# fnordware/j2k

Hardware: AMD Instinct MI355X
Metric: Mpixels/s encode, 8Kx8K 16-bit RGB, 5 DWT levels; DWT HBM GB/s vs roofline (higher is better)
Workload: dtype f32

## Files before the change

j2k_amd/csrc/t1.hip:

```cpp
#include "kernels.h"
#include "t1_common.h"
#include "cblk_style.h"
#include "t1_mq_window.h"

#include <algorithm>
#include <cstdlib>
#include <type_traits>

namespace j2k_hip {
namespace {


constexpr int kFrac = 6;
constexpr int kFlush = 1024;
constexpr int kStageBytes = kFlush + 64 * 10;


__device__ __forceinline__ void set_priority(int p)
{
    if (p >= 3) __builtin_amdgcn_s_setprio(3);
    else if (p == 2) __builtin_amdgcn_s_setprio(2);
    else if (p == 1) __builtin_amdgcn_s_setprio(1);
}

// ... 474 lines not shown
                }
                const unsigned bitsh = hf(bits), Nh = hf(A) & ~hf(O), Vh = hf(V64);
                const bool any_rl = __any(rl != 0);
                unsigned fills = 0;
                if (any_rl) {
                    unsigned nof = Nh | (Nh >> 1);
                    nof = (nof | (nof >> 2) | ~rl) & 0x11111111u;
                    int wv = w;
                    asm volatile("" : "+s"(wv));
                    if (lane >= wv) nof = 0;
#define J2K_OR_STEP(ctrl, rmask) nof |= (unsigned)__builtin_amdgcn_update_dpp(0, (int)nof, ctrl, rmask, 0xf, false);
                    J2K_OR_STEP(0x111, 0xf) J2K_OR_STEP(0x112, 0xf) J2K_OR_STEP(0x114, 0xf) J2K_OR_STEP(0x118, 0xf)
                    J2K_OR_STEP(0x142, 0xa) J2K_OR_STEP(0x143, 0xc)
#undef J2K_OR_STEP
                    fills = active & ~(unsigned)__builtin_amdgcn_readlane((int)nof, 63);
                    DADD(48, __builtin_popcount(fills));
                    if (fills == active) DCNT(49);
                }
                bool sparse = false;
                u64 q0 = 0, q1 = 0;
                unsigned sparse_total = 0;
                if (a.sparse >= 0 && !any_rl) {
                    const unsigned dense_cost = kDenseStripe * (unsigned)__builtin_popcount(active);
                    if (a.sparse > 0 || !__any(kSparseHead + kSparseRound * (unsigned)__builtin_popcount(Vh) >= dense_cost)) {
                        const unsigned c = nibble_counts(Vh) + nibble_counts(Nh);
                        const unsigned c0 = c & 0x000f000fu, c1 = (c >> 4) & 0x000f000fu, c2 = (c >> 8) & 0x000f000fu, c3 = (c >> 12) & 0x000f000fu;
                        unsigned t0, t1, t2, t3;
                        const unsigned e0 = prefix_count_dpp(c0, t0), e1 = prefix_count_dpp(c1, t1), e2 = prefix_count_dpp(c2, t2), e3 = prefix_count_dpp(c3, t3);
                        const unsigned a1 = t0 + t1, a2 = a1 + t2, a3 = a2 + t3;
                        const unsigned total = (a3 & 0xffffu) + (a3 >> 16);
                        if (total <= kBurst) {
                            sparse = true;
                            sparse_total = total;
                            DCNT(pt == 0 ? 7 : 8);
                            DADD(pt == 0 ? 14 : 15, total);
                            const unsigned org = (fill - flushed) * 0x10001u + (a3 << 16);
                            q0 = (u64)(e0 + org) | ((u64)(e1 + org + t0) << 32);
                            q1 = (u64)(e2 + org + a1) | ((u64)(e3 + org + a2) << 32);
                        } else DCNT(17);
                    }
                }
                unsigned zb0 = 0, zb1 = 0, zb2 = 0, zb3 = 0, sb0 = 0, sb1 = 0, sb2 = 0, sd = 0;
                if (fills != active) {
                    const unsigned Wm1 = hf(LA << 1), W0 = hf(LA), Wp1 = hf(((LA >> 1) & ~M3) | (LO >> 1));
                    const unsigned Em1 = hf((RO << 1) | ((RA << 1) & M0)), E0 = hf(RO), Ep1 = hf(RO >> 1);
                    const unsigned Up = hf(A << 1), Dn = hf(O >> 1);
                    {
                        unsigned h1 = W0 ^ E0, h2 = W0 & E0, v1 = Up ^ Dn, v2 = Up & Dn;
                        if (orient == 1) { const unsigned t1 = h1, t2 = h2; h1 = v1; h2 = v2; v1 = t1; v2 = t2; }
                        const unsigned p = Wm1 ^ Wp1, q = Wm1 & Wp1, r_ = Em1 ^ Ep1, t = Em1 & Ep1;
                        const unsigned dodd = p ^ r_, dge1 = p | q | r_ | t, dge2 = (p & r_) | q | t;
                        const unsigned deq1 = dodd & ~dge2;
                        const unsigned hz = ~(h1 | h2), vnz = v1 | v2;
                        if (orient == 3) {
                            const unsigned dge3 = (q & (r_ | t)) | (t & p);
                            const unsigned deq2 = dge2 & ~dge3, deq0 = ~dge1;
                            const unsigned hv0 = hz & ~vnz, hv1 = (h1 & ~vnz) | (hz & v1), hvge2 = ~(hv0 | hv1);
                            zb3 = dge3;
                            zb2 = deq2 | (deq1 & ~hv0);
                            zb1 = deq2 | (deq1 & hv0) | (deq0 & hvge2);
                            zb0 = (deq2 & ~hv0) | (deq1 & (hv0 | hvge2)) | (deq0 & hv1);
                        } else {
                            zb3 = h2;
                            zb2 = h1 | (hz & v2);
                            zb1 = (h1 & (vnz | dge1)) | (hz & (v1 | (~vnz & dge2)));
                            zb0 = (h1 & (vnz | ~dge1)) | (hz & (v1 | (~vnz & deq1)));
                        }
                    }
                    if (any_n) {
                        const unsigned cL = hf(from_left64(chi)), cR = hf(from_right64(chi)), cU = hf(chi << 1), cD = hf(chi >> 1);
                        const unsigned Wp = W0 & ~cL, Wn = W0 & cL, Ep = E0 & ~cR, En = E0 & cR;
                        const unsigned Upp = Up & ~cU, Upn = Up & cU, Dnp = Dn & ~cD, Dnn = Dn & cD;
                        const unsigned hp = (Wp & ~En) | (Ep & ~Wn), hn = (Wn & ~Ep) | (En & ~Wp);
                        const unsigned vp = (Upp & ~Dnn) | (Dnp & ~Upn), vn = (Upn & ~Dnp) | (Dnn & ~Upp);
                        const unsigned hnz = hp | hn, vnz = vp | vn;
                        const unsigned same = (hp & vp) | (hn & vn), opp = (hp & vn) | (hn & vp);
                        sb2 = same;
                        sb1 = hnz & ~same;
                        sb0 = (hnz & ~same & ~opp) | (~hnz & vnz);
                        sd = hf(chi) ^ (hn | (~hnz & vn));
                        if constexpr (BYPASS) {
                            if (pt == 0 && pass >= 10) sd = hf(chi);
                        }
                    }
                }
                if (sparse) {
                    unsigned rest = Vh, pos = 0;
                    int cur = -1;
                    while (__any(rest != 0)) {
                        DCNT(9);
                        if (rest) {
                            const int r = __builtin_ctz(rest);
                            rest &= rest - 1;
                            const int st = r >> 2;
                            if (st != cur) pos = (unsigned)((r & 8 ? q1 : q0) >> (((r & 4) << 3) | (r & 16))) & 0xffffu;
                            cur = st;
                            const auto bit = [&](unsigned plane) { return __builtin_amdgcn_ubfe(plane, (unsigned)r, 1u); };
                            stage[pos] = (unsigned char)((((((((bit(zb3) << 1) | bit(zb2)) << 1) | bit(zb1)) << 1) | bit(zb0)) << 1) | bit(bitsh));
                            ++pos;
                            if (bit(Nh)) {
                                stage[pos] = (unsigned char)(0x12u + ((((((bit(sb2) << 1) | bit(sb1)) << 1) | bit(sb0)) << 1) | bit(sd)));
                                ++pos;
                            }
                        }
                    }
                    commit(sparse_total);
                    continue;
                }
                DCNT(pt == 0 ? 12 : 13);
                unsigned zi0e = 0, zi0o = 0, zi1e = 0, zi1o = 0;
                if (kPairTabs && fills != active) {
                    pair_index(bitsh, zb0, zi0e, zi0o);
                    pair_index(zb1, zb2, zi1e, zi1o);
                }
                while (active) {
                    const int sl = __builtin_ctz(active) & ~3;
                    active &= active - 1;
                    if ((fills >> sl) & 1u) {
                        int wv = w;
                        asm volatile("" : "+s"(wv));
                        if (lane < wv) stage[(fill - flushed) + lane] = (unsigned char)(CTX_RL << 1);
                        DADD(15, w);
                        commit((unsigned)w);
                        continue;
                    }
                    DCNT(pt == 0 ? 0 : 2);
                    const unsigned N = (Nh >> sl) & 0xfu;
                    unsigned Vz = (Vh >> sl) & 0xfu;
                    unsigned pc = 0, rlsym = 0;
                    if (pt != 0) {
                        if ((rl >> sl) & 1u) {
                            const int runlen = N ? __ffs((int)N) - 1 : 4;
                            rlsym = (CTX_RL << 1) | (runlen != 4 ? 1u : 0u);
                            pc = 1;
                            Vz = 0;
                            if (runlen != 4) {
                                rlsym |= (((CTX_UNI << 1) | (unsigned)(runlen >> 1)) << 8) | (((CTX_UNI << 1) | (unsigned)(runlen & 1)) << 16);
                                pc = 3;
                                Vz = 0xfu & ~((2u << runlen) - 1u);
                            }
                        }
                    }
                    const u64 sel = DIST ? kPackSel.v[Vz | (N << 4)] : sel_tab[Vz | (N << 4)];
                    const unsigned cnt = pc + (unsigned)__builtin_popcount(Vz) + (unsigned)__builtin_popcount(N);
                    unsigned total;
                    const unsigned base = reserve(cnt, std::integral_constant<int, 10>(), total);
                    unsigned zsym = 0, ssym = 0;
                    const auto nib = [&](unsigned plane) { return __builtin_amdgcn_ubfe(plane, (unsigned)sl, 4u); };
                    if constexpr (kPairTabs) {
                        const unsigned pick = 0x0c0c0c00u | ((unsigned)sl >> 3) | ((unsigned)sl & 4u);
                        if (__any(Vz != 0))
                            zsym = pair_entry(__builtin_amdgcn_perm(zi0o, zi0e, pick)) | (pair_entry(__builtin_amdgcn_perm(zi1o, zi1e, pick)) << 2) |
                                   (spread4(nib(zb3)) << 4);
                        if (__any(N != 0))
                            ssym = 0x12121212u + pair_entry(nib(sd) | (nib(sb0) << 4)) + (pair_entry(nib(sb1) | (nib(sb2) << 4)) << 2);
                    } else {
                        if (__any(Vz != 0))
                            zsym = (spread4(nib(zb0)) << 1) | (spread4(nib(zb1)) << 2) | (spread4(nib(zb2)) << 3) | (spread4(nib(zb3)) << 4) | spread4(nib(bitsh));
                        if (__any(N != 0))
                            ssym = 0x12121212u + (spread4(nib(sb0)) << 1) + (spread4(nib(sb1)) << 2) + (spread4(nib(sb2)) << 3) + spread4(nib(sd));
                    }
                    {
                        const unsigned c0 = __builtin_amdgcn_perm(ssym, zsym, (unsigned)sel), c1 = __builtin_amdgcn_perm(ssym, zsym, (unsigned)(sel >> 32));
                        const u64 d = (((u64)c1 << 32) | c0) << (8 * pc);
                        emit(base, cnt, (unsigned)d | rlsym, (unsigned)(d >> 32), __builtin_amdgcn_ubfe(c1, 8, 8 * pc));
                        DADD(pt == 0 ? 14 : 15, total);
                        commit(total);
                    }
                }
            }
            sigma = A;
            }
            }
            if (pt == 2) pi = 0;
            if constexpr (DIST) {
#pragma unroll
                for (int o = 32; o > 0; o >>= 1) nm += __shfl_xor(nm, o);
            }
            if (lane == 0) { pass_nsym[pass] = fill; pass_nmsedec[pass] = nm; }
            ++pass;
        }
    }
    __builtin_amdgcn_wave_barrier();
    const unsigned rest = fill - flushed;
    if (lane * 16u < rest) {
        if (flushed + lane * 16u + 16u <= symcap) {
            const uint4 v = *reinterpret_cast<const uint4 *>(&stage[lane * 16]);
            *reinterpret_cast<uint4 *>(symout + flushed + lane * 16) = v;
        } else overflow = true;
    }
#ifdef J2K_T1_COUNTERS
    if (lane == 0 && a.dbg) for (int i = 0; i < kT1Counters; ++i) if (dc[i]) atomicAdd(a.dbg + i, dc[i]);
#endif
    const bool ovf = __any(overflow);
    if (ovf && lane == 0) a.err[0] = 2u;
    if (lane == 0) { a.numbps[b] = (unsigned)numbps; a.npasses[b] = ovf ? 0u : (unsigned)pass; a.nsym[b] = ovf ? 0u : fill; }
    report();
}

constexpr unsigned mq2_slot(unsigned idx, unsigned mps, unsigned lps) { return idx | (mps << 6) | (lps << 7); }
constexpr unsigned kMq2LpsBit = 9;
constexpr bool mq2_slots_ok()
{
    bool seen[256] = {};
    for (unsigned idx = 0; idx < 47; ++idx)
        for (unsigned mps = 0; mps < 2; ++mps)
            for (unsigned lps = 0; lps < 2; ++lps) {
                const unsigned w = mq2_slot(idx, mps, lps), addr = w * 4u;
                if (w >= 256u || seen[w] || (addr & 3u) || (addr & ~0x3fcu)) return false;
                if (addr != ((mq2_slot(idx, mps, 0) * 4u) ^ (lps << kMq2LpsBit))) return false;
                seen[w] = true;
            }
    return true;
}
static_assert(mq2_slots_ok(), "trans: (index, sense, lps) -> word index must be injective over 47 x 2 x 2, below 256, and a word address within 0x3fc");
__device__ __forceinline__ unsigned ctx_word2(unsigned qe, unsigned idx, unsigned mps) { return (qe << 16) | (mq2_slot(idx, mps, 0) << 2) | (mps << kMq2LpsBit); }

#ifndef J2K_MQ2_RING
#define J2K_MQ2_RING 128
#endif
constexpr unsigned kRing = J2K_MQ2_RING;
template <bool RATES>
__global__ __launch_bounds__(128) void t1_mq2_kernel(T1Args a)
{
    __shared__ unsigned ctxs[19 * 64];
    __shared__ unsigned trans[256];
    __shared__ uint4 queue[2][4][64];
    __shared__ __attribute__((aligned(16))) unsigned ostage[(kRing / 4 + 1) * 64];
    __shared__ unsigned finalA[64];
    const int lane = threadIdx.x & 63;
    const bool producer = threadIdx.x < 64;
    __shared__ int gate_ok;
    T1Args::GateGroup gg{};
    bool gated_out = false;
    if (a.gate_groups) {
        gg = a.gate_groups[a.first + (int)blockIdx.x];
        if (threadIdx.x == 0) {
            unsigned polls = 0;
            int ok = 1;
            while (__hip_atomic_load(a.gate_ready + a.first + (int)blockIdx.x, __ATOMIC_ACQUIRE, __HIP_MEMORY_SCOPE_AGENT) < gg.count) {
                __builtin_amdgcn_s_sleep(127);
                if (++polls > a.gate_budget || (a.gate_abort && __hip_atomic_load(a.gate_abort, __ATOMIC_RELAXED, __HIP_MEMORY_SCOPE_AGENT))) { ok = 0; break; }
            }
            gate_ok = ok;
        }
        __syncthreads();
        __builtin_amdgcn_fence(__ATOMIC_ACQUIRE, "agent");
        gated_out = gate_ok == 0;
        if (gated_out && threadIdx.x == 0) a.err[0] = 4u;
        set_priority(a.mq_prio ? (int)gg.prio : 0);
    } else set_priority(a.mq_prio);
    const int b = a.gate_groups ? (int)gg.first + lane : a.first + (int)blockIdx.x * 64 + lane;
    if (producer) {
        if (lane < 47) {
            trans[mq2_slot(lane, 0, 0)] = ctx_word2(kQe[kNmps[lane]], kNmps[lane], 0);
            trans[mq2_slot(lane, 1, 0)] = ctx_word2(kQe[kNmps[lane]], kNmps[lane], 1);
            trans[mq2_slot(lane, 0, 1)] = ctx_word2(kQe[kNlps[lane]], kNlps[lane], kSwitch[lane]);
            trans[mq2_slot(lane, 1, 1)] = ctx_word2(kQe[kNlps[lane]], kNlps[lane], 1u ^ kSwitch[lane]);
        }
#pragma unroll
        for (int c = 0; c < 19; ++c) {
            const unsigned idx = c == CTX_UNI ? 46u : (c == CTX_RL ? 3u : (c == 0 ? 4u : 0u));
            ctxs[c * 64 + lane] = ctx_word2(kQe[idx], idx, 0);
        }
    }
    const bool live = a.gate_groups ? (lane < (int)gg.count && !gated_out) : b < a.nblks;
    CblkDev cb = {};
    unsigned nsym = 0, npasses = 0;
    if (live) { cb = a.blks[b]; nsym = a.nsym[b]; npasses = a.npasses[b]; }
    unsigned maxsym = nsym;
#pragma unroll
    for (int o = 32; o > 0; o >>= 1) maxsym = max(maxsym, (unsigned)__shfl_xor((int)maxsym, o));
    const unsigned nchunks = (unsigned)__builtin_amdgcn_readfirstlane((int)((maxsym + 15) / 16));
    __syncthreads();

    if (producer) {
        const unsigned char *sym = a.sym + cb.sym_off;
        unsigned A = 0x80000000u;
        uint4 next = make_uint4(0, 0, 0, 0);
        if (nsym) next = *reinterpret_cast<const uint4 *>(sym);
        unsigned yield_budget = 2048;
#ifdef J2K_MQ_TIMES
        long long tw_ = 0, tb_ = 0;
#endif
        for (unsigned c = 0; c <= nchunks; ++c) {
#ifdef J2K_MQ_TIMES
            const long long t0_ = __builtin_readcyclecounter();
#endif
            if (a.yield_word && (c & 3u) == 0) {
                while (yield_budget && __builtin_amdgcn_readfirstlane((int)__hip_atomic_load(a.yield_word, __ATOMIC_RELAXED, __HIP_MEMORY_SCOPE_AGENT))) {
                    __builtin_amdgcn_s_sleep(64);
                    --yield_budget;
                }
            }
            if (c < nchunks) {
                const unsigned base = c * 16;
                const uint4 chunk = next;
                if (base + 16 < nsym) next = *reinterpret_cast<const uint4 *>(sym + base + 16);
                const unsigned words[4] = {chunk.x, chunk.y, chunk.z, chunk.w};
                const int rem = (int)min(nsym - min(base, nsym), 16u);
                unsigned char *const ctx_b = reinterpret_cast<unsigned char *>(ctxs);
                const unsigned char *const trans_b = reinterpret_cast<const unsigned char *>(trans);
                const unsigned lane4 = (unsigned)lane * 4u;
                auto decide = [&](unsigned c4, unsigned b4, auto jj_) -> unsigned {
                    constexpr unsigned jj = decltype(jj_)::value;
                    unsigned *const cp = reinterpret_cast<unsigned *>(ctx_b + __builtin_amdgcn_perm(c4, lane4, 0x0c0c0400u + (jj << 8)));
                    const unsigned st = *cp;
                    const unsigned ta = (st ^ __builtin_amdgcn_perm(b4, 0u, 0x0c0c040cu + (jj << 8))) & 0x3fcu;
                    const unsigned tr = *reinterpret_cast<const unsigned *>(trans_b + ta);
                    const bool mps = ta < (1u << kMq2LpsBit);
                    const unsigned qe = st & 0xffff0000u;
                    const unsigned A1 = A - qe;
                    const bool use_a1 = (A1 >= qe) == mps;
                    A = use_a1 ? A1 : qe;
                    const bool renorm = (int)A >= 0;
                    *cp = renorm ? tr : st;
                    const unsigned n = (unsigned)__builtin_clz(A);
                    A <<= n;
                    return __builtin_amdgcn_alignbit(n, use_a1 ? qe : 0u, 16);
                };
                if (__all(rem == 16)) {
#pragma unroll
                    for (int g = 0; g < 4; ++g) {
                        const unsigned c4 = (words[g] >> 1) & 0x1f1f1f1fu, b4 = words[g] << 1;
                        unsigned e[4];
                        e[0] = decide(c4, b4, std::integral_constant<unsigned, 0>());
                        e[1] = decide(c4, b4, std::integral_constant<unsigned, 1>());
                        e[2] = decide(c4, b4, std::integral_constant<unsigned, 2>());
                        e[3] = decide(c4, b4, std::integral_constant<unsigned, 3>());
                        queue[c & 1][g][lane] = make_uint4(e[0], e[1], e[2], e[3]);
                    }
                } else
#pragma unroll
                for (int g = 0; g < 4; ++g) {
                    const unsigned c4 = (words[g] >> 1) & 0x1f1f1f1fu, b4 = words[g] << 1;
                    unsigned e[4] = {0, 0, 0, 0};
                    if (4 * g + 0 < rem) e[0] = decide(c4, b4, std::integral_constant<unsigned, 0>());
                    if (4 * g + 1 < rem) e[1] = decide(c4, b4, std::integral_constant<unsigned, 1>());
                    if (4 * g + 2 < rem) e[2] = decide(c4, b4, std::integral_constant<unsigned, 2>());
                    if (4 * g + 3 < rem) e[3] = decide(c4, b4, std::integral_constant<unsigned, 3>());
                    queue[c & 1][g][lane] = make_uint4(e[0], e[1], e[2], e[3]);
                }
            } else {
                finalA[lane] = A >> 16;
            }
#ifdef J2K_MQ_TIMES
            const long long t1_ = __builtin_readcyclecounter();
            __syncthreads();
            tw_ += t1_ - t0_; tb_ += __builtin_readcyclecounter() - t1_;
#else
            __syncthreads();
#endif
        }
#ifdef J2K_MQ_TIMES
        if (lane == 0 && a.dbg) { atomicAdd(a.dbg + 0, (unsigned long long)tw_); atomicAdd(a.dbg + 1, (unsigned long long)tb_); atomicAdd(a.dbg + 4, (unsigned long long)nchunks); atomicAdd(a.dbg + 5, 1ull); }
#endif
        return;
    }

    unsigned char *out = a.out + cb.out_off;
    const unsigned *pass_nsym = a.pass_nsym + (size_t)(live ? b : 0) * kDevMaxPasses;
    unsigned *pass_rate = a.pass_rate + (size_t)(live ? b : 0) * kDevMaxPasses;
    unsigned char *ostage_b = reinterpret_cast<unsigned char *>(ostage);
    unsigned C = 0, CT = 12, B = 0;
    bool window = false, window_again = false;
    if constexpr (!RATES) { window = a.mq_window >= 0; window_again = a.mq_window == 2; }
    MqWide wide = mq_wide_from(C, CT, B);
    int flushed = 0;
    bool overflow = false;
    const unsigned dbase = (unsigned)lane * (kRing + 4u) + 4u;
    unsigned pos = dbase - 1u;
    auto nbytes = [&]() -> int { return (int)(pos - dbase) + flushed; };
    auto byteout = [&](bool p) {
        const bool was_ff = B == 0xffu;
        const unsigned Bc = B + ((C > 0x7ffffffu && !was_ff) ? 1u : 0u);
        const bool stuff = Bc == 0xffu;
        const unsigned sh = stuff ? 20u : 19u, ct = 27u - sh;
        const unsigned bw = was_ff ? 8u : ct;
        ostage_b[pos] = (unsigned char)Bc;
        B = p ? __builtin_amdgcn_ubfe(C, sh, bw) : B; C = p ? __builtin_amdgcn_ubfe(C, 0u, sh) : C; CT = p ? ct : CT; pos += p ? 1u : 0u;
        asm("" : "+v"(pos));
    };
    unsigned cur_pass = 0;
    unsigned next_end = 0xffffffffu;
    if constexpr (RATES) next_end = npasses ? pass_nsym[0] : 0xffffffffu;
    auto close_passes = [&](unsigned i) {
        while (cur_pass < npasses && i == next_end) {
            pass_rate[cur_pass] = (unsigned)(nbytes() + 3);
            ++cur_pass;
            next_end = cur_pass < npasses ? pass_nsym[cur_pass] : 0xffffffffu;
        }
    };
#ifdef J2K_MQ_TIMES
    long long tw_ = 0, tb_ = 0;
#endif
    for (unsigned c = 0; c <= nchunks; ++c) {
#ifdef J2K_MQ_TIMES
        const long long t0_ = __builtin_readcyclecounter();
#endif
        if (c >= 1) {
            const unsigned base = (c - 1) * 16;
            int rel = 64;
            if constexpr (RATES) rel = (int)min(next_end - base, 64u);
            auto four = [&](auto check, const unsigned (&e)[4], const int g) {
                constexpr bool ENDS = decltype(check)::value;
                {
#pragma unroll
                    for (int jj = 0; jj < 4; ++jj) {
                        const int j = 4 * g + jj;
                        C += e[jj] & 0xffffu;
                        unsigned n = e[jj] >> 16;
                        {
                            const bool p = n >= CT;
                            const unsigned k = p ? CT : 0u;
                            C <<= k; n -= k;
                            byteout(p);
                        }
                        if (__any(n >= CT)) {
                            const bool p2 = n >= CT;
                            const unsigned k2 = p2 ? CT : 0u;
                            C <<= k2; n -= k2;
                            byteout(p2);
                            if (__any(n >= CT)) {
                                const bool p3 = n >= CT;
                                const unsigned k3 = p3 ? CT : 0u;
                                C <<= k3; n -= k3;
                                byteout(p3);
                            }
                        }
                        C <<= n; CT -= n;
                        if constexpr (ENDS) {
                            if (rel == j + 1) { close_passes(base + j + 1); rel = (int)min(next_end - base, 64u); }
                        }
                    }
                }
            };
            bool ends_here = false;
            if constexpr (RATES) ends_here = __any(rel <= 16);
#pragma unroll
            for (int g = 0; g < 4; ++g) {
                const uint4 q = queue[(c - 1) & 1][g][lane];
                const unsigned e[4] = {q.x, q.y, q.z, q.w};
                if constexpr (RATES) {
                    if (ends_here && __any(rel > 4 * g && rel <= 4 * g + 4)) four(std::true_type(), e, g);
                    else four(std::false_type(), e, g);
                } else if (window) {
                    const MqWide wide0 = wide;
                    const unsigned pos0 = pos;
#pragma unroll
                    for (int jj = 0; jj < 4; ++jj) mq_wide_add(wide, e[jj]);
                    bool again = window_again || mq_wide_is_wide(wide) || mq_wide_has_carry(wide);
                    if (!__any(again)) {
                        while (__any(mq_wide_due(wide))) {
                            const bool due = mq_wide_due(wide);
                            const unsigned byte = mq_wide_peel(wide, due, again);
                            ostage_b[pos] = (unsigned char)byte;
                            pos += due ? 1u : 0u;
                        }
                    }
                    if (__any(again)) {
                        pos = pos0;
                        mq_wide_to(wide0, C, CT, B);
                        four(std::false_type(), e, g);
                        wide = mq_wide_from(C, CT, B);
                    }
                } else four(std::false_type(), e, g);
            }
            const int waiting = (int)(pos - dbase);
            if (__any(waiting >= 64)) {
                const int units = waiting >> 4;
                for (int u = 0; u < 7; ++u) {
                    if (!__any(u < units)) break;
                    if (u < units) {
                        if ((unsigned)(flushed + 16) <= cb.out_cap) {
                            const unsigned *sp = reinterpret_cast<const unsigned *>(ostage_b + dbase + 16 * u);
                            *reinterpret_cast<uint4 *>(out + flushed) = make_uint4(sp[0], sp[1], sp[2], sp[3]);
                        } else overflow = true;
                        flushed += 16;
                    }
                }
                if (units > 0) {
                    const unsigned *sp = reinterpret_cast<const unsigned *>(ostage_b + dbase + 16 * units);
                    unsigned *dp = reinterpret_cast<unsigned *>(ostage_b + dbase);
                    const unsigned r0 = sp[0], r1 = sp[1], r2 = sp[2], r3 = sp[3];
                    dp[0] = r0; dp[1] = r1; dp[2] = r2; dp[3] = r3;
                    pos -= 16u * (unsigned)units;
                }
            }
        }
#ifdef J2K_MQ_TIMES
        const long long t1_ = __builtin_readcyclecounter();
        __syncthreads();
        tw_ += t1_ - t0_; tb_ += __builtin_readcyclecounter() - t1_;
#else
        __syncthreads();
#endif
    }
#ifdef J2K_MQ_TIMES
    if (lane == 0 && a.dbg) { atomicAdd(a.dbg + 2, (unsigned long long)tw_); atomicAdd(a.dbg + 3, (unsigned long long)tb_); }
#endif
    if constexpr (!RATES) {
        if (window) mq_wide_to(wide, C, CT, B);
    }
    const bool fin = live && npasses;
    const unsigned A = finalA[lane];
    if (fin) {
        if constexpr (RATES) close_passes(nsym);
        const unsigned tempc = C + A;
        C |= 0xffffu;
        if (C >= tempc) C -= 0x8000u;
    }
    C <<= CT; byteout(fin);
    C <<= CT; byteout(fin);
    if (fin && B != 0xffu) {
        ostage_b[pos] = (unsigned char)B;
        ++pos;
    }
    const int nb = nbytes();
    if (fin) {
        for (int o = flushed; o < nb; o += 4) {
            if ((unsigned)(o + 4) <= cb.out_cap) *reinterpret_cast<unsigned *>(out + o) = *reinterpret_cast<const unsigned *>(ostage_b + dbase + (o - flushed));
            else overflow = true;
        }
        if constexpr (RATES) pass_rate[npasses - 1] = (unsigned)nb;
        a.len[b] = (unsigned)nb;
        if (overflow) a.err[0] = 3u;
    } else if (live) {
        a.len[b] = 0;
    } else if (a.gate_groups && lane < (int)gg.count) {
        a.len[b] = 0;
    }
    if (a.gate_groups) {
        __builtin_amdgcn_fence(__ATOMIC_RELEASE, "agent");
        if (lane == 0) __hip_atomic_fetch_add(a.gate_done + gg.stage, 1u, __ATOMIC_RELEASE, __HIP_MEMORY_SCOPE_AGENT);
    }
}

__global__ void t1_rate_fixup_kernel(T1Args a)
{
    const int b = a.first + (int)(blockIdx.x * blockDim.x + threadIdx.x);
    if (b >= a.nblks) return;
    const unsigned np = a.npasses[b];
    unsigned *rate = a.pass_rate + (size_t)b * kDevMaxPasses;
    const unsigned char *bytes = a.out + a.blks[b].out_off;
    unsigned last = a.len[b];
    for (unsigned p = np; p > 0;) { --p; if (rate[p] > last) rate[p] = last; else last = rate[p]; }
    for (unsigned p = 0; p < np; ++p)
        if (rate[p] > 0 && bytes[rate[p] - 1] == 0xffu) --rate[p];
}

__global__ void wait_word_kernel(const unsigned *word, unsigned target, unsigned timeout_us)
{
    for (unsigned i = 0; i < timeout_us; ++i) {
        if ((int)(__hip_atomic_load(word, __ATOMIC_RELAXED, __HIP_MEMORY_SCOPE_AGENT) - target) >= 0) return;
        __builtin_amdgcn_s_sleep(32);
    }
}

__global__ void wait_count_kernel(const unsigned *word, unsigned target, unsigned timeout_us, const unsigned *abort, unsigned *err)
{
    for (unsigned i = 0; i < timeout_us; i += 2) {
        if (__hip_atomic_load(word, __ATOMIC_ACQUIRE, __HIP_MEMORY_SCOPE_AGENT) >= target) return;
        if (abort && __hip_atomic_load(abort, __ATOMIC_RELAXED, __HIP_MEMORY_SCOPE_AGENT)) break;
        __builtin_amdgcn_s_sleep(64);
    }
    if (threadIdx.x == 0) *err = 5u;
}

__global__ void set_word_kernel(unsigned *word, unsigned value, unsigned *word2, unsigned value2)
{
    if (threadIdx.x == 0) {
        if (word2) __hip_atomic_store(word2, value2, __ATOMIC_RELAXED, __HIP_MEMORY_SCOPE_AGENT);
        __hip_atomic_store(word, value, __ATOMIC_RELAXED, __HIP_MEMORY_SCOPE_AGENT);
    }
}

}

void launch_wait_word(const unsigned *word, unsigned target, unsigned timeout_us, hipStream_t s)
{
    hipLaunchKernelGGL(wait_word_kernel, dim3(1), dim3(64), 0, s, word, target, timeout_us);
}

void launch_wait_count(const unsigned *word, unsigned target, unsigned timeout_us, const unsigned *abort, unsigned *err, hipStream_t s)
{
    hipLaunchKernelGGL(wait_count_kernel, dim3(1), dim3(64), 0, s, word, target, timeout_us, abort, err);
}

void launch_set_word(unsigned *word, unsigned value, hipStream_t s, unsigned *word2, unsigned value2)
{
    hipLaunchKernelGGL(set_word_kernel, dim3(1), dim3(64), 0, s, word, value, word2, value2);
}

void launch_t1_rate_fixup(const T1Args &a, hipStream_t s)
{
    const int n = a.nblks - a.first;
    if (n <= 0) return;
    hipLaunchKernelGGL(t1_rate_fixup_kernel, dim3((unsigned)((n + 63) / 64)), dim3(64), 0, s, a);
}

void launch_t1_model(const T1Args &a, hipStream_t s)
{
    const int n = a.nblks - a.first;
    if (n <= 0) return;
    if (a.want_dist) {
        if (a.reversible) hipLaunchKernelGGL((t1_model_kernel<true, true>), dim3((unsigned)n), dim3(64), 0, s, a);
        else hipLaunchKernelGGL((t1_model_kernel<false, true>), dim3((unsigned)n), dim3(64), 0, s, a);
    } else if (a.style & kStyleBypass) {
        if (a.reversible) hipLaunchKernelGGL((t1_model_kernel<true, false, true>), dim3((unsigned)n), dim3(64), 0, s, a);
        else hipLaunchKernelGGL((t1_model_kernel<false, false, true>), dim3((unsigned)n), dim3(64), 0, s, a);
    } else {
        if (a.reversible) hipLaunchKernelGGL((t1_model_kernel<true, false>), dim3((unsigned)n), dim3(64), 0, s, a);
        else hipLaunchKernelGGL((t1_model_kernel<false, false>), dim3((unsigned)n), dim3(64), 0, s, a);
    }
}

void launch_t1_mq_gated(const T1Args &a, int group_first, int group_count, hipStream_t s)
{
    if (group_count <= 0 || !a.gate_groups) return;
    T1Args g = a;
    g.first = group_first;
    if (g.want_rates) hipLaunchKernelGGL(t1_mq2_kernel<true>, dim3((unsigned)group_count), dim3(128), 0, s, g);
    else hipLaunchKernelGGL(t1_mq2_kernel<false>, dim3((unsigned)group_count), dim3(128), 0, s, g);
}

void launch_t1_mq(const T1Args &a, hipStream_t s)
{
    const int n = a.nblks - a.first;
    if (n <= 0) return;
    if (a.style) { launch_t1_mq_styled(a, s); return; }
    if (a.want_rates) hipLaunchKernelGGL(t1_mq2_kernel<true>, dim3((unsigned)((n + 63) / 64)), dim3(128), 0, s, a);
    else hipLaunchKernelGGL(t1_mq2_kernel<false>, dim3((unsigned)((n + 63) / 64)), dim3(128), 0, s, a);
}

}
```

j2k_amd/csrc/t1_mq_window.h:

```cpp
#pragma once

#if defined(__HIPCC__)
#define J2K_WIN_HD __host__ __device__ __forceinline__
#else
#define J2K_WIN_HD inline
#endif

namespace j2k_hip {

struct MqWide {
    unsigned long long V;
    unsigned w;
};

constexpr unsigned kMqWideDue = 8u + 27u;
constexpr unsigned kMqWideMax = 63u;

J2K_WIN_HD MqWide mq_wide_from(unsigned C, unsigned CT, unsigned B)
{
    MqWide s;
    s.V = ((unsigned long long)B << (27u - CT)) + C;
    s.w = kMqWideDue - CT;
    return s;
}
J2K_WIN_HD void mq_wide_to(const MqWide &s, unsigned &C, unsigned &CT, unsigned &B)
{
    const unsigned k = s.w - 8u;
    const unsigned top = (unsigned)(s.V >> k), over = top >> 8;
    CT = kMqWideDue - s.w;
    B = top - over;
    C = ((unsigned)s.V & ((1u << k) - 1u)) | (over << k);
}

J2K_WIN_HD void mq_wide_add(MqWide &s, unsigned e)
{
    const unsigned n = e >> 16;
    s.V = (s.V + (e & 0xffffu)) << n;
    s.w += n;
}

J2K_WIN_HD bool mq_wide_is_wide(const MqWide &s) { return s.w > kMqWideMax; }
J2K_WIN_HD bool mq_wide_has_carry(const MqWide &s) { return (s.V >> (s.w & 63u)) != 0; }

J2K_WIN_HD bool mq_wide_due(const MqWide &s) { return s.w >= kMqWideDue; }
J2K_WIN_HD unsigned mq_wide_peel(MqWide &s, bool p, bool &rolled)
{
    const unsigned k = s.w - 8u;
    const unsigned byte = (unsigned)(s.V >> k);
    const unsigned long long rest = s.V - ((unsigned long long)byte << k);
    const unsigned w1 = s.w - (byte == 0xffu ? 7u : 8u);
    const bool zero = (rest >> (w1 - 8u)) == 0;
    s.V = p ? rest : s.V;
    s.w = p ? w1 : s.w;
    rolled = rolled || (p && zero);
    return byte;
}

}
```

Baseline: 11340.

## Pre-reduce MQ decisions into per-group sums and bound peel rounds in window path

```diff
diff --git a/j2k_amd/csrc/t1.hip b/j2k_amd/csrc/t1.hip
--- a/j2k_amd/csrc/t1.hip
+++ b/j2k_amd/csrc/t1.hip
@@ -800,7 +800,7 @@
                 unsigned char *const ctx_b = reinterpret_cast<unsigned char *>(ctxs);
                 const unsigned char *const trans_b = reinterpret_cast<const unsigned char *>(trans);
                 const unsigned lane4 = (unsigned)lane * 4u;
-                auto decide = [&](unsigned c4, unsigned b4, auto jj_) -> unsigned {
+                auto decide = [&](unsigned c4, unsigned b4, auto jj_, unsigned &q, unsigned &nn) -> unsigned {
                     constexpr unsigned jj = decltype(jj_)::value;
                     unsigned *const cp = reinterpret_cast<unsigned *>(ctx_b + __builtin_amdgcn_perm(c4, lane4, 0x0c0c0400u + (jj << 8)));
                     const unsigned st = *cp;
@@ -815,29 +815,63 @@
                     *cp = renorm ? tr : st;
                     const unsigned n = (unsigned)__builtin_clz(A);
                     A <<= n;
-                    return __builtin_amdgcn_alignbit(n, use_a1 ? qe : 0u, 16);
+                    if constexpr (RATES) return __builtin_amdgcn_alignbit(n, use_a1 ? qe : 0u, 16);
+                    q = use_a1 ? qe : 0u;
+                    nn = n;
+                    return 0u;
+                };
+                auto send = [&](const int g, const unsigned (&q)[4], const unsigned (&n)[4]) {
+                    unsigned G = 0, N = 0, shifts = 0;
+#pragma unroll
+                    for (int jj = 0; jj < 4; ++jj) {
+                        mq_group_add(G, N, q[jj] >> 16, n[jj]);
+                        shifts = mq_group_add_shift(shifts, n[jj], (unsigned)jj);
+                    }
+                    uint2 *const half = reinterpret_cast<uint2 *>(queue) + ((c & 1) * 4 + g) * 128 + lane;
+                    half[0] = make_uint2(G, shifts);
+                    half[64] = make_uint2(mq_group_pack_addends_high(q[0], q[1]), mq_group_pack_addends_high(q[2], q[3]));
                 };
                 if (__all(rem == 16)) {
 #pragma unroll
                     for (int g = 0; g < 4; ++g) {
                         const unsigned c4 = (words[g] >> 1) & 0x1f1f1f1fu, b4 = words[g] << 1;
-                        unsigned e[4];
-                        e[0] = decide(c4, b4, std::integral_constant<unsigned, 0>());
-                        e[1] = decide(c4, b4, std::integral_constant<unsigned, 1>());
-                        e[2] = decide(c4, b4, std::integral_constant<unsigned, 2>());
-                        e[3] = decide(c4, b4, std::integral_constant<unsigned, 3>());
-                        queue[c & 1][g][lane] = make_uint4(e[0], e[1], e[2], e[3]);
+                        unsigned e[4], q[4], n[4];
+                        e[0] = decide(c4, b4, std::integral_constant<unsigned, 0>(), q[0], n[0]);
+                        e[1] = decide(c4, b4, std::integral_constant<unsigned, 1>(), q[1], n[1]);
+                        e[2] = decide(c4, b4, std::integral_constant<unsigned, 2>(), q[2], n[2]);
+                        e[3] = decide(c4, b4, std::integral_constant<unsigned, 3>(), q[3], n[3]);
+                        if constexpr (RATES) queue[c & 1][g][lane] = make_uint4(e[0], e[1], e[2], e[3]);
+                        else send(g, q, n);
                     }
                 } else
 #pragma unroll
                 for (int g = 0; g < 4; ++g) {
                     const unsigned c4 = (words[g] >> 1) & 0x1f1f1f1fu, b4 = words[g] << 1;
-                    unsigned e[4] = {0, 0, 0, 0};
-                    if (4 * g + 0 < rem) e[0] = decide(c4, b4, std::integral_constant<unsigned, 0>());
-                    if (4 * g + 1 < rem) e[1] = decide(c4, b4, std::integral_constant<unsigned, 1>());
-                    if (4 * g + 2 < rem) e[2] = decide(c4, b4, std::integral_constant<unsigned, 2>());
-                    if (4 * g + 3 < rem) e[3] = decide(c4, b4, std::integral_constant<unsigned, 3>());
-                    queue[c & 1][g][lane] = make_uint4(e[0], e[1], e[2], e[3]);
+                    if constexpr (RATES) {
+                        unsigned e[4] = {0, 0, 0, 0}, q, n;
+                        if (4 * g + 0 < rem) e[0] = decide(c4, b4, std::integral_constant<unsigned, 0>(), q, n);
+                        if (4 * g + 1 < rem) e[1] = decide(c4, b4, std::integral_constant<unsigned, 1>(), q, n);
+                        if (4 * g + 2 < rem) e[2] = decide(c4, b4, std::integral_constant<unsigned, 2>(), q, n);
+                        if (4 * g + 3 < rem) e[3] = decide(c4, b4, std::integral_constant<unsigned, 3>(), q, n);
+                        queue[c & 1][g][lane] = make_uint4(e[0], e[1], e[2], e[3]);
+                    } else {
+                        unsigned G = 0, N = 0, shifts = 0, a[2] = {0, 0};
+                        auto one = [&](auto jj_) {
+                            constexpr unsigned jj = decltype(jj_)::value;
+                            unsigned q, n;
+                            decide(c4, b4, jj_, q, n);
+                            mq_group_add(G, N, q >> 16, n);
+                            shifts = mq_group_add_shift(shifts, n, jj);
+                            a[jj >> 1] = (jj & 1u) ? mq_group_pack_addends(a[jj >> 1], q >> 16) : q >> 16;
+                        };
+                        if (4 * g + 0 < rem) one(std::integral_constant<unsigned, 0>());
+                        if (4 * g + 1 < rem) one(std::integral_constant<unsigned, 1>());
+                        if (4 * g + 2 < rem) one(std::integral_constant<unsigned, 2>());
+                        if (4 * g + 3 < rem) one(std::integral_constant<unsigned, 3>());
+                        uint2 *const half = reinterpret_cast<uint2 *>(queue) + ((c & 1) * 4 + g) * 128 + lane;
+                        half[0] = make_uint2(G, shifts);
+                        half[64] = make_uint2(a[0], a[1]);
+                    }
                 }
             } else {
                 finalA[lane] = A >> 16;
@@ -861,8 +895,8 @@
     unsigned *pass_rate = a.pass_rate + (size_t)(live ? b : 0) * kDevMaxPasses;
     unsigned char *ostage_b = reinterpret_cast<unsigned char *>(ostage);
     unsigned C = 0, CT = 12, B = 0;
-    bool window = false, window_again = false;
-    if constexpr (!RATES) { window = a.mq_window >= 0; window_again = a.mq_window == 2; }
+    bool window = false, window_again = false, window_long = false;
+    if constexpr (!RATES) { window = a.mq_window >= 0; window_again = a.mq_window == 2; window_long = a.mq_window == 3; }
     MqWide wide = mq_wide_from(C, CT, B);
     int flushed = 0;
     bool overflow = false;
@@ -937,32 +971,53 @@
             if constexpr (RATES) ends_here = __any(rel <= 16);
 #pragma unroll
             for (int g = 0; g < 4; ++g) {
-                const uint4 q = queue[(c - 1) & 1][g][lane];
-                const unsigned e[4] = {q.x, q.y, q.z, q.w};
                 if constexpr (RATES) {
+                    const uint4 q = queue[(c - 1) & 1][g][lane];
+                    const unsigned e[4] = {q.x, q.y, q.z, q.w};
                     if (ends_here && __any(rel > 4 * g && rel <= 4 * g + 4)) four(std::true_type(), e, g);
                     else four(std::false_type(), e, g);
-                } else if (window) {
+                } else {
+                    const uint2 *const half = reinterpret_cast<const uint2 *>(queue) + (((c - 1) & 1) * 4 + g) * 128 + lane;
+                    uint2 q = half[0];
+                    asm("" : "+v"(q.x), "+v"(q.y));
+                    bool again = true;
                     const MqWide wide0 = wide;
                     const unsigned pos0 = pos;
-#pragma unroll
-                    for (int jj = 0; jj < 4; ++jj) mq_wide_add(wide, e[jj]);
-                    bool again = window_again || mq_wide_is_wide(wide) || mq_wide_has_carry(wide);
-                    if (!__any(again)) {
-                        while (__any(mq_wide_due(wide))) {
-                            const bool due = mq_wide_due(wide);
-                            const unsigned byte = mq_wide_peel(wide, due, again);
-                            ostage_b[pos] = (unsigned char)byte;
-                            pos += due ? 1u : 0u;
+                    if (window) {
+                        const unsigned N = mq_group_N(q.y);
+                        mq_wide_add_group(wide, q.x, N);
+                        again = __any(window_long || mq_group_is_long(N) || mq_wide_has_carry(wide));
+                        if (!again) {
+                            const unsigned long long V_after = wide.V;
+                            unsigned zpos = kMqNoZero;
+                            static_assert(kMqExactMax + kMqGroupMaxN - 3u * 7u < kMqWideDue, "three peel rounds must do");
+                            auto round = [&]() {
+                                const bool due = mq_wide_due(wide);
+                                const unsigned byte = mq_wide_peel_mark(wide, due, zpos);
+                                ostage_b[pos] = (unsigned char)byte;
+                                pos += due ? 1u : 0u;
+                            };
+                            if (__any(mq_wide_due(wide))) {
+                                round();
+                                if (__any(mq_wide_due(wide))) {
+                                    round();
+                                    if (__any(mq_wide_due(wide))) round();
+                                }
+                            }
+                            again = window_again;
+                            if (__any(zpos != kMqNoZero)) again = __any(window_again || mq_group_rolled(V_after, wide0.V, N, zpos));
                         }
                     }
-                    if (__any(again)) {
-                        pos = pos0;
-                        mq_wide_to(wide0, C, CT, B);
+                    if (again) {
+                        const uint2 r = half[64];
+                        unsigned e[4];
+#pragma unroll
+                        for (unsigned jj = 0; jj < 4; ++jj) e[jj] = mq_group_decision(q.y, r.x, r.y, jj);
+                        if (window) { pos = pos0; mq_wide_to(wide0, C, CT, B); }
                         four(std::false_type(), e, g);
-                        wide = mq_wide_from(C, CT, B);
-                    }
-                } else four(std::false_type(), e, g);
+                        if (window) wide = mq_wide_from(C, CT, B);
+                    }
+                }
             }
             const int waiting = (int)(pos - dbase);
             if (__any(waiting >= 64)) {
diff --git a/j2k_amd/csrc/t1_mq_window.h b/j2k_amd/csrc/t1_mq_window.h
--- a/j2k_amd/csrc/t1_mq_window.h
+++ b/j2k_amd/csrc/t1_mq_window.h
@@ -56,4 +56,71 @@
     return byte;
 }
 
+constexpr unsigned kMqAddendMax = 0x5601u;
+constexpr unsigned kMqGroupMaxN = 15u;
+constexpr unsigned kMqExactMax = kMqWideDue - 1u;
+static_assert(((4ull * kMqAddendMax) << kMqGroupMaxN) < (1ull << 32), "G of a group that is not long must fit 32 bits");
+static_assert(((4ull * kMqAddendMax) << (kMqGroupMaxN + 1u)) >= (1ull << 32), "(and one shift more does not: the bound is tight)");
+static_assert(kMqExactMax + kMqGroupMaxN <= kMqWideMax, "a group that is not long cannot be wide");
+
+J2K_WIN_HD void mq_group_add(unsigned &G, unsigned &N, unsigned addend, unsigned n)
+{
+    G = (G + addend) << n;
+    N += n;
 }
+J2K_WIN_HD bool mq_group_is_long(unsigned N) { return N > kMqGroupMaxN; }
+J2K_WIN_HD void mq_wide_add_group(MqWide &s, unsigned G, unsigned N)
+{
+    s.V = (s.V << N) + G;
+    s.w += N;
+}
+
+J2K_WIN_HD unsigned mq_group_pack_shifts(unsigned n0, unsigned n1, unsigned n2, unsigned n3, unsigned N)
+{
+    return n0 | (n1 << 4) | (n2 << 8) | (n3 << 12) | (N << 16);
+}
+J2K_WIN_HD unsigned mq_group_add_shift(unsigned shifts, unsigned n, unsigned jj)
+{
+    const unsigned k = (1u << (4u * jj)) | 0x10000u;
+#if defined(__HIP_DEVICE_COMPILE__)
+    return __umul24(n, k) + shifts;
+#else
+    return n * k + shifts;
+#endif
+}
+J2K_WIN_HD unsigned mq_group_pack_addends(unsigned first, unsigned second) { return first | (second << 16); }
+J2K_WIN_HD unsigned mq_group_pack_addends_high(unsigned first, unsigned second)
+{
+#if defined(__HIP_DEVICE_COMPILE__)
+    return __builtin_amdgcn_perm(second, first, 0x07060302u);
+#else
+    return (first >> 16) | (second & 0xffff0000u);
+#endif
+}
+J2K_WIN_HD unsigned mq_group_N(unsigned shifts) { return shifts >> 16; }
+J2K_WIN_HD unsigned mq_group_decision(unsigned shifts, unsigned a01, unsigned a23, unsigned jj)
+{
+    const unsigned pair = jj < 2u ? a01 : a23;
+    const unsigned addend = (jj & 1u) ? pair >> 16 : pair & 0xffffu;
+    return addend | (((shifts >> (4u * jj)) & 15u) << 16);
+}
+
+constexpr unsigned kMqNoZero = 63u;
+J2K_WIN_HD unsigned mq_wide_peel_mark(MqWide &s, bool p, unsigned &zpos)
+{
+    const unsigned k = s.w - 8u;
+    const unsigned byte = (unsigned)(s.V >> k);
+    const unsigned long long rest = s.V - ((unsigned long long)byte << k);
+    const unsigned w1 = s.w - (byte == 0xffu ? 7u : 8u);
+    const bool zero = (rest >> (w1 - 8u)) == 0;
+    s.V = p ? rest : s.V;
+    s.w = p ? w1 : s.w;
+    zpos = (p && zero) ? k : zpos;
+    return byte;
+}
+J2K_WIN_HD bool mq_group_rolled(unsigned long long V_after, unsigned long long V_start, unsigned N, unsigned zpos)
+{
+    return zpos != kMqNoZero && ((V_after ^ (V_start << N)) >> zpos) != 0;
+}
+
+}
```

After: 11750 (median of 6 runs). 1.04x the previous value.
